# tudelft-iv/CCVPE

Measured on AMD Instinct MI355X. Metric: image-pairs/sec, higher is better.
Workload: dtype f32

## Files before the change

### ccvpe_amd/csrc/tail512.hip

```cpp
#include "conv_common.h"

namespace ccvpe {

struct TailParams {
  const void* x;
  const void* w;
  const float* shift9;
  const float* w2;
  const float* b2;
  float* out;
  float* smx;
  int H1, W1, c0, ld0, Kpad, normalize;
  int tiles_x, tiles_y, tiles_total, tiles_per_wg;
};

template <typename T, int COUT, int NCH, int TY, int TX, int WPP, bool SPLIT = false, bool PERSIST = false>
struct TailGeom {
  static constexpr int NW = 4 * WPP;
  static constexpr int NTHR = 64 * NW;
  static constexpr int PW = TX + 1;
  static constexpr int P = (TY + 1) * PW;
  static constexpr int NTILE = (P + 15) / 16;
  static constexpr int TPW = (NTILE + WPP - 1) / WPP;
  static constexpr int HR = TY + 2, HC = TX + 2, HPX = HR * HC;
  static constexpr bool WIDE_SLOT = TY == 8 && TX == 16 && (SPLIT || sizeof(T) == 2);
  static constexpr int LD = WIDE_SLOT ? 24 : 20;
  static constexpr int HCP = WIDE_SLOT ? 25 : HC;
  static constexpr int XBUF = HR * HCP * LD;
  static constexpr int NXB = NCH > 1 ? 2 : 1;
  static constexpr int SH = 2 * TY + 2, SW = 2 * TX + 2, SPL = SH * SW;
  static constexpr int NPL = 10;
  static constexpr int MAIN = (NXB * XBUF > NPL * SPL) ? NXB * XBUF : NPL * SPL;
  static constexpr int LDS_BYTES = (MAIN + 9 * 16) * 4;
  static constexpr int NOUT = (4 * TY * TX) / NTHR;
};

__device__ __forceinline__ void split4(f32x4 v, bf16x4& hi, bf16x4& lo) {
#pragma unroll
  for (int i = 0; i < 4; ++i) {
    hi[i] = (bf16_t)v[i];
    lo[i] = (bf16_t)(v[i] - (float)hi[i]);
  }
}

template <typename T, int COUT, int NCH, int TY, int TX, int WPP, bool SPLIT, bool PERSIST>
__global__ __launch_bounds__(256 * WPP, 2) void tail512_kernel(const TailParams p) {
  static_assert(!SPLIT || sizeof(T) == 4, "SPLIT reads fp32 operands");
  using G = TailGeom<T, COUT, NCH, TY, TX, WPP, SPLIT, PERSIST>;
  constexpr int E = ElemTraits<T>::E;
  constexpr int SK = 4 * E;
  constexpr int NTHR = G::NTHR, PW = G::PW, P = G::P, TPW = G::TPW;
  constexpr int HC = G::HC, HCP = G::HCP, HPX = G::HPX, LD = G::LD, XBUF = G::XBUF;
  constexpr int SW = G::SW, SPL = G::SPL;
  constexpr int H_IT = (HPX * 4 + NTHR - 1) / NTHR;
  static_assert((4 * TY * TX) % NTHR == 0, "stage 3 hands every thread the same number of outputs");

  extern __shared__ __attribute__((aligned(16))) float t5_sm[];
  float* Xs = t5_sm;
  float* Sp = t5_sm;
  float* Sh9 = t5_sm + G::MAIN;

  const int tid = threadIdx.x;
  const int lane = tid & 63;
  const int wave = sgpr(tid >> 6);
  const int par = wave & 3, wsub = wave >> 2;
  const int py = par >> 1, px = par & 1;
  const int pix = lane & 15, q = lane >> 4;

  const int wg = xcd_tile(blockIdx.x, gridDim.x);
  const int t_begin = wg * p.tiles_per_wg;
  const int t_end = min(t_begin + p.tiles_per_wg, p.tiles_total);
  const int tiles_xy = p.tiles_x * p.tiles_y;
  int b, y0, x0;
  auto tile_coords = [&](int t, int& tb, int& ty0, int& tx0) {
    tb = t / tiles_xy;
    const int r = t - tb * tiles_xy;
    const int ty = r / p.tiles_x;
    ty0 = ty * TY;
    tx0 = (r - ty * p.tiles_x) * TX;
  };
  const int H2 = 2 * p.H1, W2 = 2 * p.W1;
  const T* xg = reinterpret_cast<const T*>(p.x);

  for (int i = tid; i < 9 * 16; i += NTHR) Sh9[i] = p.shift9[i];

  constexpr int NWR = SPLIT ? 2 : 1;
  f32x4 wr[4][NCH][NWR];
  if constexpr (!SPLIT) {
    const T* wp = reinterpret_cast<const T*>(p.w) + ((size_t)par * 16 + pix) * p.Kpad;
#pragma unroll
    for (int tap = 0; tap < 4; ++tap)
#pragma unroll
      for (int c = 0; c < NCH; ++c) {
        const int ch = c * SK + q * E;
        wr[tap][c][0] = *reinterpret_cast<const f32x4*>(wp + (ch < p.c0 ? tap * p.c0 + ch : 0));
      }
#pragma unroll
    for (int tap = 0; tap < 4; ++tap)
#pragma unroll
      for (int c = 0; c < NCH; ++c) wr[tap][c][0] = keep_if(wr[tap][c][0], c * SK + q * E < p.c0);
  } else {
    const float* wp = reinterpret_cast<const float*>(p.w) + ((size_t)par * 16 + pix) * p.Kpad;
#pragma unroll
    for (int tap = 0; tap < 4; ++tap)
#pragma unroll
      for (int c = 0; c < NCH; ++c) {
        const int ch = c * 16 + (q & 1) * 8;
        const bool ok = ch < p.c0;
        const f32x4 v0 = keep_if(*reinterpret_cast<const f32x4*>(wp + (ok ? tap * p.c0 + ch : 0)), ok);
        const f32x4 v1 = keep_if(*reinterpret_cast<const f32x4*>(wp + (ok ? tap * p.c0 + ch + 4 : 0)), ok);
        bf16x4 h0, l0, h1, l1;
        split4(v0, h0, l0);
        split4(v1, h1, l1);
        bf16x8 hi, lo;
#pragma unroll
        for (int i = 0; i < 4; ++i) { hi[i] = h0[i]; hi[i + 4] = h1[i]; lo[i] = l0[i]; lo[i + 4] = l1[i]; }
        wr[tap][c][0] = __builtin_bit_cast(f32x4, hi);
        wr[tap][c][1] = keep_if(__builtin_bit_cast(f32x4, lo), q < 2);
      }
  }
  f32x4 w2f[COUT];
#pragma unroll
  for (int o = 0; o < COUT; ++o) {
    w2f[o] = keep_if(*reinterpret_cast<const f32x4*>(p.w2 + (o * 9 + min(pix, 8)) * 16 + q * 4), pix < 9);
  }

  const int hsub = tid & 3;
  int tidv = tid;
  f32x4 h_reg[H_IT];
  unsigned h_keep = 0;
  const int ld0s = sgpr(p.ld0);
  auto load_halo = [&](int c, int hb, int hy0, int hx0) {
    const int ch = c * SK + hsub * E;
    h_keep = 0;
#pragma unroll
    for (int it = 0; it < H_IT; ++it) {
      const int pxl = (tidv + NTHR * it) >> 2;
      const int hy = pxl / HC, hx = pxl - hy * HC;
      const int iy = hy0 - 1 + hy, ix = hx0 - 1 + hx;
      const bool ok = pxl < HPX && (unsigned)iy < (unsigned)p.H1 && (unsigned)ix < (unsigned)p.W1 && ch < p.c0;
      h_reg[it] = *reinterpret_cast<const f32x4*>(xg + (ok ? (size_t)((hb * p.H1 + iy) * p.W1 + ix) * ld0s + ch : 0));
      h_keep |= ok ? (1u << it) : 0u;
    }
  };
  auto store_halo = [&](int buf) {
#pragma unroll
    for (int it = 0; it < H_IT; ++it) {
      const int pxl = (tidv + NTHR * it) >> 2;
      const int slot = HCP == HC ? pxl : (pxl / HC) * HCP + (pxl % HC);
      const f32x4 v = keep_if(h_reg[it], (h_keep >> it) & 1u);
      if constexpr (!SPLIT) {
        if (pxl < HPX) *reinterpret_cast<f32x4*>(Xs + buf * XBUF + slot * LD + hsub * 4) = v;
      } else {
        bf16x4 hi, lo;
        split4(v, hi, lo);
        if (pxl < HPX) {
          float* row = Xs + buf * XBUF + slot * LD;
          *reinterpret_cast<bf16x4*>(reinterpret_cast<bf16_t*>(row) + hsub * 4) = hi;
          *reinterpret_cast<bf16x4*>(reinterpret_cast<bf16_t*>(row) + 16 + hsub * 4) = lo;
        }
      }
    }
  };

  if (t_begin >= t_end) return;
  tile_coords(t_begin, b, y0, x0);
  load_halo(0, b, y0, x0);
  for (int t = t_begin; t < t_end; ++t) {
  asm volatile("v_mov_b32 %0, %0" : "+v"(tidv));
  const int pixv = tidv & 15, qv = (tidv >> 4) & 3;
  int fbase[TPW];
#pragma unroll
  for (int i = 0; i < TPW; ++i) {
    const int pc = min((wsub * TPW + i) * 16 + pixv, P - 1);
    const int iy = pc / PW, ix = pc - iy * PW;
    fbase[i] = (iy * HCP + ix) * LD + qv * 4;
  }
  f32x4 acc[TPW];
#pragma unroll
  for (int i = 0; i < TPW; ++i) acc[i] = (f32x4){0.f, 0.f, 0.f, 0.f};

  store_halo(0);
  __syncthreads();
  constexpr int NPAIR = (TPW + 1) / 2, NS = NPAIR * 4;
#pragma unroll
  for (int c = 0; c < NCH; ++c) {
    if (c + 1 < NCH) load_halo(c + 1, b, y0, x0);
    __builtin_amdgcn_sched_barrier(0);
    const float* xb = Xs + (c & 1) * XBUF;
    f32x4 fr[2][2];
    auto read_step = [&](int s, f32x4* dst) {
      const int g = s >> 2, tap = s & 3;
      const int toff = ((tap >> 1) * HCP + (tap & 1)) * LD;
      dst[0] = *reinterpret_cast<const f32x4*>(xb + fbase[2 * g] + toff);
      if (2 * g + 1 < TPW) dst[1] = *reinterpret_cast<const f32x4*>(xb + fbase[2 * g + 1] + toff);
    };
    read_step(0, fr[0]);
#pragma unroll
    for (int s = 0; s < NS; ++s) {
      const int g = s >> 2, tap = s & 3;
      if (s + 1 < NS) read_step(s + 1, fr[(s + 1) & 1]);
      __builtin_amdgcn_sched_barrier(0);
      const f32x4 wv = wr[tap][c][0];
      const f32x4 f0 = fr[s & 1][0], f1 = fr[s & 1][1];
      if constexpr (SPLIT) {
#pragma unroll
        for (int h = 0; h < 2; ++h) {
          acc[2 * g] = mfma_stage<bf16_t>(wr[tap][c][h], f0, acc[2 * g]);
          if (2 * g + 1 < TPW) acc[2 * g + 1] = mfma_stage<bf16_t>(wr[tap][c][h], f1, acc[2 * g + 1]);
        }
      } else if constexpr (sizeof(T) == 4) {
#pragma unroll
        for (int kk = 0; kk < 4; ++kk) {
          acc[2 * g] = __builtin_amdgcn_mfma_f32_16x16x4f32(wv[kk], f0[kk], acc[2 * g], 0, 0, 0);
          if (2 * g + 1 < TPW) acc[2 * g + 1] = __builtin_amdgcn_mfma_f32_16x16x4f32(wv[kk], f1[kk], acc[2 * g + 1], 0, 0, 0);
        }
      } else {
        acc[2 * g] = mfma_stage<T>(wv, f0, acc[2 * g]);
        if (2 * g + 1 < TPW) acc[2 * g + 1] = mfma_stage<T>(wv, f1, acc[2 * g + 1]);
      }
      __builtin_amdgcn_sched_barrier(0);
    }
    if (c + 1 < NCH) {
      store_halo((c + 1) & 1);
      __syncthreads();
    }
  }
  if constexpr (PERSIST) {
    int nb, ny0, nx0;
    tile_coords(min(t + 1, t_end - 1), nb, ny0, nx0);
    load_halo(0, nb, ny0, nx0);
  }
  __syncthreads();
  __builtin_amdgcn_sched_barrier(0);

#pragma unroll
  for (int i = 0; i < TPW; ++i) {
    const int pc = min((wsub * TPW + i) * 16 + pixv, P - 1);
    const int iy = pc / PW, ix = pc - iy * PW;
    const int Y = 2 * (y0 + iy) - py, X = 2 * (x0 + ix) - px;
    const bool inside = (unsigned)Y < (unsigned)H2 && (unsigned)X < (unsigned)W2;
    const int rc = Y <= 0 ? 0 : (Y >= H2 - 1 ? 2 : 1);
    const int cc = X <= 0 ? 0 : (X >= W2 - 1 ? 2 : 1);
    const f32x4 sh = *reinterpret_cast<const f32x4*>(Sh9 + (rc * 3 + cc) * 16 + qv * 4);
#pragma unroll
    for (int r = 0; r < 4; ++r) acc[i][r] = inside ? fmaxf(acc[i][r] + sh[r], 0.f) : 0.f;
  }
  float res[COUT][G::NOUT];
#pragma unroll
  for (int o = 0; o < COUT; ++o) {
#pragma unroll
    for (int i = 0; i < TPW; ++i) {
      f32x4 s = {0.f, 0.f, 0.f, 0.f};
#pragma unroll
      for (int r = 0; r < 4; ++r) s = __builtin_amdgcn_mfma_f32_16x16x4f32(w2f[o][r], acc[i][r], s, 0, 0, 0);
      const int pt = (wsub * TPW + i) * 16 + pixv;
      const int iy = pt / PW, ix = pt - iy * PW;
      float* dst = Sp + (2 * iy + 1 - py) * SW + (2 * ix + 1 - px);
      if (pt < P) {
#pragma unroll
        for (int r = 0; r < 4; ++r) dst[min(4 * qv + r, 9) * SPL] = s[r];
      }
    }
    __syncthreads();
#pragma unroll
    for (int k = 0; k < G::NOUT; ++k) {
      const int e = tidv + NTHR * k;
      const int Yo = e / (2 * TX), Xo = e - Yo * (2 * TX);
      float v = p.b2[o];
#pragma unroll
      for (int t = 0; t < 9; ++t) v += Sp[t * SPL + (Yo + t / 3) * SW + Xo + t % 3];
      res[o][k] = v;
    }
    if (o + 1 < COUT) __syncthreads();
  }
#pragma unroll
  for (int k = 0; k < G::NOUT; ++k) {
    const int e = tidv + NTHR * k;
    const int Yo = e / (2 * TX), Xo = e - Yo * (2 * TX);
    if (COUT == 2 && p.normalize) {
      const float n = fmaxf(sqrtf(res[0][k] * res[0][k] + res[COUT - 1][k] * res[COUT - 1][k]), 1e-12f);
      res[0][k] /= n;
      res[COUT - 1][k] /= n;
    }
#pragma unroll
    for (int o = 0; o < COUT; ++o)
      p.out[((size_t)(b * COUT + o) * H2 + 2 * y0 + Yo) * W2 + 2 * x0 + Xo] = res[o][k];
  }
  if (COUT == 1 && p.smx) {
    float m = res[0][0];
#pragma unroll
    for (int k = 1; k < G::NOUT; ++k) m = fmaxf(m, res[0][k]);
    m = wave_max(m);
    float e = 0.f;
#pragma unroll
    for (int k = 0; k < G::NOUT; ++k) e += expf(res[0][k] - m);
    e = wave_sum(e);
    if (lane == 0) {
      float* dst = p.smx + ((size_t)t * G::NW + wave) * 2;
      dst[0] = m;
      dst[1] = e;
    }
  }
  if constexpr (!PERSIST) break;
  tile_coords(min(t + 1, t_end - 1), b, y0, x0);
  __syncthreads();
  }
}

template <typename T, int COUT, int NCH, int TY, int TX, int WPP, bool SPLIT = false, bool PERSIST = false>
static int launch_tail(const TailParams& p0, int batch, hipStream_t stream) {
  using G = TailGeom<T, COUT, NCH, TY, TX, WPP, SPLIT, PERSIST>;
  TailParams p = p0;
  if (p.W1 % TX || p.H1 % TY) return fail(CCVPE_EINVAL, "tail512: %d x %d is not a multiple of the %d x %d tile", p.H1, p.W1, TY, TX);
  p.tiles_x = p.W1 / TX;
  p.tiles_y = p.H1 / TY;
  const long total = (long)p.tiles_x * p.tiles_y * batch;
  if (total <= 0 || total > 0x7fffffffL) return fail(CCVPE_EINVAL, "tail512: bad grid");
  p.tiles_total = (int)total;
  const int max_wgs = 256 * 2 * 8;
  p.tiles_per_wg = PERSIST ? (int)((total + max_wgs - 1) / max_wgs) : 1;
  const int wgs = (int)((total + p.tiles_per_wg - 1) / p.tiles_per_wg);
  static bool attr_set = false;
  if (!attr_set) {
    hipError_t e = hipFuncSetAttribute((const void*)tail512_kernel<T, COUT, NCH, TY, TX, WPP, SPLIT, PERSIST>,
                                       hipFuncAttributeMaxDynamicSharedMemorySize, G::LDS_BYTES);
    if (e != hipSuccess) return fail(CCVPE_ELAUNCH, "tail512: set smem attr: %s", hipGetErrorString(e));
    attr_set = true;
  }
  hipLaunchKernelGGL((tail512_kernel<T, COUT, NCH, TY, TX, WPP, SPLIT, PERSIST>), dim3(wgs), dim3(G::NTHR), G::LDS_BYTES, stream, p);
  return check_launch("tail512_kernel");
}

template <typename T>
static int tail_any(const ccvpe_tail_desc* d, void* stream) {
  constexpr int E = ElemTraits<T>::E;
  constexpr int SK = 4 * E;
  if (!d) return fail(CCVPE_EINVAL, "tail512: null desc");
  if (d->c0 <= 0 || d->c0 % 8 || d->ld0 % E || d->ld0 < d->c0) return fail(CCVPE_EINVAL, "tail512: c0 %% 8, ld0 %% %d, ld0 >= c0 required", E);
  if (d->kpad < 4 * d->c0) return fail(CCVPE_EINVAL, "tail512: kpad %d < 4 * c0", d->kpad);
  if (d->cout != 1 && d->cout != 2) return fail(CCVPE_EINVAL, "tail512: cout must be 1 or 2");
  if (!d->x || !d->w || !d->shift9 || !d->w2 || !d->b2 || !d->out) return fail(CCVPE_EINVAL, "tail512: null pointer");
  if (!aligned16(d->x) || !aligned16(d->w) || !aligned16(d->w2) || !aligned16(d->shift9))
    return fail(CCVPE_EINVAL, "tail512: pointers must be 16-byte aligned");
  if (d->batch <= 0 || d->h1 <= 0 || d->w1 <= 0 || (long)d->batch * d->h1 * d->w1 > 0x1fffffffL) return fail(CCVPE_EINVAL, "tail512: bad shape");
  if (d->h1 % 16 || d->w1 % 16) return fail(CCVPE_EINVAL, "tail512: h1 and w1 must be multiples of 16 (got %d x %d)", d->h1, d->w1);
  TailParams p;
  p.x = d->x; p.w = d->w; p.shift9 = d->shift9; p.w2 = d->w2; p.b2 = d->b2; p.out = d->out;
  p.smx = d->cout == 1 ? d->softmax_partial : nullptr;
  p.H1 = d->h1; p.W1 = d->w1; p.c0 = d->c0; p.ld0 = d->ld0; p.Kpad = d->kpad; p.normalize = d->normalize;
  p.tiles_x = p.tiles_y = p.tiles_total = p.tiles_per_wg = 0;
  const int nch = (d->c0 + SK - 1) / SK;
  hipStream_t st = (hipStream_t)stream;
#define CCVPE_TAIL(COUT_, NCH_)                                                                                \
  if (d->cout == COUT_ && nch == NCH_) {                                                                       \
    if constexpr (sizeof(T) == 4) return launch_tail<T, COUT_, NCH_, 16, 16, 1, false, false>(p, d->batch, st); \
    else return launch_tail<T, COUT_, NCH_, 8, 16, 1, false, true>(p, d->batch, st);                           \
  }
  if constexpr (sizeof(T) == 4) {
    if (d->split) {
      if (d->cout == 1 && nch == 2) return launch_tail<T, 1, 2, 8, 16, 1, true, true>(p, d->batch, st);
      if (d->cout == 1 && nch == 3) return launch_tail<T, 1, 3, 8, 16, 1, true, true>(p, d->batch, st);
      return fail(CCVPE_EINVAL, "tail512: split mode is instantiated for cout 1, 17..48 channels");
    }
    CCVPE_TAIL(1, 2) CCVPE_TAIL(1, 3) CCVPE_TAIL(2, 2)
  } else {
    if (d->split) return fail(CCVPE_EINVAL, "tail512: split mode takes fp32 operands");
    CCVPE_TAIL(1, 1) CCVPE_TAIL(1, 2) CCVPE_TAIL(2, 1)
  }
#undef CCVPE_TAIL
  return fail(CCVPE_EINVAL, "tail512: (cout %d, c0 %d) not instantiated (fp32: cout 1 with c0 <= 48, cout 2 with c0 <= 32; bf16: cout 1 "
                            "with c0 <= 64, cout 2 with c0 <= 32)", d->cout, d->c0);
}

template <typename T>
static int tail_partials(const ccvpe_tail_desc* d) {
  if (!d || d->h1 <= 0 || d->w1 <= 0) return fail(CCVPE_EINVAL, "tail512_partials: bad desc");
  const bool small = sizeof(T) == 2 || d->split;
  const int ty = small ? 8 : 16;
  if (d->h1 % ty || d->w1 % 16) return fail(CCVPE_EINVAL, "tail512_partials: shape not tiled");
  return (d->h1 / ty) * (d->w1 / 16) * 4;
}

}

using namespace ccvpe;

extern "C" int ccvpe_tail512_partials(const ccvpe_tail_desc* desc, int is_bf16) {
  return is_bf16 ? tail_partials<bf16_t>(desc) : tail_partials<float>(desc);
}
extern "C" int ccvpe_tail512_f32(const ccvpe_tail_desc* desc, void* stream) { return tail_any<float>(desc, stream); }
extern "C" int ccvpe_tail512_bf16(const ccvpe_tail_desc* desc, void* stream) { return tail_any<bf16_t>(desc, stream); }
```

### ccvpe_amd/models.py

```python
import torch
import torch.nn as nn

from . import ops
from .synth import B0_BLOCKS, MODEL_SPECS, state_dict_spec

BN_EPS = 1e-3
SKIP_BLOCKS = (15, 10, 4, 2, 0)
MATCH_STRIDES = {"vigor": (64, 32, 16, 8, 4, 2),
                 "kitti": (128, 64, 32, 16, 8, 8),
                 "oxford": (64, 32, 16, 8, 4, 2)}


def window_offset(kind, channels, length):
    return int(channels / 2 - length / 2) if kind == "oxford" else 0


def _round_up(v, m):
    return (v + m - 1) // m * m


class _Holder(nn.Module):

    def forward(self, *a, **k):
        raise RuntimeError("parameter holder is not callable; use the owning CVM_* module")
# ... 59 lines not shown
def _pack_encoder(sd, p, dtype=torch.float32, fold_bn=True):
    fold = _fold_bn if fold_bn else (lambda _sd, _p: (None, None))
    e = _Obj()
    e.stem_w = sd[p + "._conv_stem.weight"].permute(2, 3, 1, 0).contiguous()
    e.stem_scale, e.stem_shift = fold(sd, p + "._bn0")
    e.blocks = []
    for i, (k, s, ex, cin, cout) in enumerate(B0_BLOCKS):
        b = _Obj()
        bp = "%s._blocks.%d" % (p, i)
        b.k, b.s, b.expand, b.cin, b.cout, b.mid = k, s, ex != 1, cin, cout, cin * ex
        if b.expand:
            b.w_exp = _pack_conv(sd[bp + "._expand_conv.weight"], dtype)
            b.s0, b.b0 = fold(sd, bp + "._bn0")
        b.w_dw = sd[bp + "._depthwise_conv.weight"].reshape(b.mid, k, k).permute(1, 2, 0).contiguous()
        b.s1, b.b1 = fold(sd, bp + "._bn1")
        b.se_w1 = sd[bp + "._se_reduce.weight"].reshape(-1, b.mid).contiguous()
        b.se_b1 = sd[bp + "._se_reduce.bias"].contiguous()
        b.se_w2 = sd[bp + "._se_expand.weight"].reshape(b.mid, -1).t().contiguous()
        b.se_b2 = sd[bp + "._se_expand.bias"].contiguous()
        b.w_proj = _pack_conv(sd[bp + "._project_conv.weight"], dtype)
        b.s2, b.b2 = fold(sd, bp + "._bn2")
        b.skip = (s == 1 and cin == cout)
        e.blocks.append(b)
    e.w_head = _pack_conv(sd[p + "._conv_head.weight"], dtype)
    e.head_scale, e.head_shift = fold(sd, p + "._bn1")
    return e


def _pack_deconv(w, bias, col_map, ldo, dtype=torch.float32):
    cin, cout = w.shape[0], w.shape[1]
    wg = w.permute(2, 3, 1, 0).reshape(4 * cout, cin)
    out = w.new_zeros((4 * cout, ldo))
    for d0, s0, n in col_map:
        out[:, d0:d0 + n] = wg[:, s0:s0 + n]
    return _pad2(out, dtype), bias.repeat(4).contiguous()


_UP_S = {0: {0: ((0, 1),), 1: ((1, 0), (2, 1))}, 1: {0: ((0, 0), (1, 1)), 1: ((2, 0),)}}
_UP_R = {0: (1, 2), 1: (0, 1, 2), 2: (0, 1)}
_OVERLAP_ENV = __import__("os").environ.get("CCVPE_OVERLAP_DECODERS", "auto")


OVERLAP_DECODERS_MAX_BATCH = 128


def _overlap_decoders(precision, batch=1):
    return _OVERLAP_ENV == "1" or (_OVERLAP_ENV == "auto" and precision == "bf16" and batch <= OVERLAP_DECODERS_MAX_BATCH)
FOLD_LEVELS = tuple(int(c) for c in __import__("os").environ.get("CCVPE_FOLD_LEVELS", "012345"))
FOLD_MIN_PIXELS = int(__import__("os").environ.get("CCVPE_FOLD_MIN_PIXELS", "2048"))
FUSE_TAIL = __import__("os").environ.get("CCVPE_FUSE_TAIL", "1") != "0"
SPLIT_TAIL = __import__("os").environ.get("CCVPE_SPLIT_TAIL", "1") != "0"
WINO = __import__("os").environ.get("CCVPE_WINO", "1") != "0"
SPLIT3 = __import__("os").environ.get("CCVPE_SPLIT3", "1") != "0"
SPLIT3_MIN_OK = 2
PACK_GRAPH = __import__("os").environ.get("CCVPE_PACK_GRAPH", "1") != "0"
PACK_GATHER = __import__("os").environ.get("CCVPE_PACK_GATHER", "1") != "0"
FUSE_MATCH = __import__("os").environ.get("CCVPE_FUSE_MATCH", "1") != "0"
FUSE_STEM = __import__("os").environ.get("CCVPE_FUSE_STEM", "1") != "0"
EVAL_TWO_STREAMS = __import__("os").environ.get("CCVPE_EVAL_TWO_STREAMS", "1") != "0"


def _pack_upconv(wd, bd, col_map, cp, w3, b3, dtype=torch.float32):
    cd, co = wd.shape[1], w3.shape[0]
    c1 = w3.shape[1] - cd
    wd_my = wd.new_zeros((cp, cd, 2, 2), dtype=torch.float64)
    for d0, s0, n in col_map:
        wd_my[d0:d0 + n] = wd[s0:s0 + n].double()
    w3d = w3[:, :cd].double()
    k = 4 * cp + 9 * c1
    kmult = 16 if dtype == torch.float32 else 32
    out = wd.new_zeros((4, _round_up(co, 16), _round_up(k, kmult)), dtype=torch.float64)
    for py in range(2):
        for px in range(2):
            par = py * 2 + px
            for du in range(2):
                for dv in range(2):
                    weff = wd.new_zeros((co, cp), dtype=torch.float64)
                    for ky, a in _UP_S[py][du]:
                        for kx, b in _UP_S[px][dv]:
                            weff += w3d[:, :, ky, kx] @ wd_my[:, :, a, b].t()
                    tap = du * 2 + dv
                    out[par, :co, tap * cp:(tap + 1) * cp] = weff
            if c1:
                out[par, :co, 4 * cp:k] = w3[:, cd:].double().permute(0, 2, 3, 1).reshape(co, 9 * c1)
    shift9 = wd.new_zeros((9, co), dtype=torch.float64)
    for rc in range(3):
        for cc in range(3):
            v = b3.double().clone()
            for ky in _UP_R[rc]:
                for kx in _UP_R[cc]:
                    v += w3d[:, :, ky, kx] @ bd.double()
            shift9[rc * 3 + cc] = v
    return out.to(dtype).contiguous(), shift9.float().contiguous()


def _split3_bf16(v):
    hi = v.to(torch.bfloat16)
    r = v - hi.float()
    mid = r.to(torch.bfloat16)
    lo = (r - mid.float()).to(torch.bfloat16)
    return hi, mid, lo


def _pack_upconv_s3(fw, cp, c1, dtype=torch.float32):
    if dtype != torch.float32 or fw is None or fw.dtype != torch.float32 or c1 <= 0:
        return None
    npad = fw.shape[1]
    nb0, nb1 = (cp + 15) // 16, (c1 + 15) // 16
    a = fw.new_zeros((4, npad, 4, nb0 * 16))
    a[..., :cp] = fw[:, :, :4 * cp].reshape(4, npad, 4, cp)
    a = a.reshape(4, npad, 4, nb0, 16).permute(0, 3, 2, 1, 4).reshape(4, 4 * nb0, npad, 16)
    s = fw.new_zeros((4, npad, 9, nb1 * 16))
# ... 258 lines not shown
            if gp is not None and gp[0] == where:
                self._pack_cache = gp[1].run()
            else:
                plan = repack.build(sd, pack)
                if plan is None:
                    self._pack_plan, self._pack_plan_failed = None, True
                    return self._packed()
                self._pack_plan = (where, plan)
                self._pack_cache = plan.pk
        elif self.training and PACK_GRAPH:
            where = (self.precision, self.fp32_tail_levels) + tuple(
                t.data_ptr() for t in list(self.parameters()) + list(self.buffers()))
            g = getattr(self, "_pack_graph", None)
            if g is not None and g[0] == where:
                g[1].replay()
                self._pack_cache = g[2]
            elif getattr(self, "_pack_where", None) == where and not getattr(self, "_pack_graph_failed", False):
                try:
                    graph = torch.cuda.CUDAGraph()
                    with torch.cuda.graph(graph, capture_error_mode="thread_local"):
                        pk = pack()
                    graph.replay()
                    self._pack_graph = (where, graph, pk)
                    self._pack_cache = pk
                except Exception:
                    self._pack_graph, self._pack_graph_failed = None, True
                    self._pack_cache = pack()
            else:
                self._pack_graph = None
                self._pack_where = where
                self._pack_cache = pack()
        else:
            self._pack_cache = pack()
        self._pack_key = key
        return self._pack_cache

    def _side_stream(self, which=1):
        dev = next(self.parameters()).device
        streams = self.__dict__.setdefault("_side_streams", {})
        st = streams.get(which)
        if st is None or st.device != dev:
            st = torch.cuda.Stream(device=dev)
            streams[which] = st
        return st

    def _ori_decoder(self, pk, cat6, sfeats, batch):
        xo = cat6
        normalize = not getattr(self, "ori_raw_output", False)
        for j in range(6):
            ov = pk.ori[j]
            hw = xo.shape[1]
            skip = sfeats[SKIP_BLOCKS[j]] if j < 5 else None
            if j == 5 and FUSE_TAIL and j in FOLD_LEVELS and ops.tail512_ok(hw, hw, ov.n_a):
                return ops.tail512(xo, ov.k, ov.fw, ov.fshift, ov.w_b, ov.b_b, 2, normalize, batch=batch, h1=hw, w1=hw)
            if j in FOLD_LEVELS and batch * hw * hw >= FOLD_MIN_PIXELS:
                y = _upconv_a(ov, xo, ov.k, batch, hw, skip)
            else:
                up = ops.conv_igemm(xo, ov.k, ov.up_w, ov.up_n, batch=batch, in_h=hw, in_w=hw,
                                    shift=ov.up_b, out_mode=ops.OUT_DECONV2X, algo_k=ov.k_algo)
                y = _double_conv(ov, up, skip, batch, 2 * hw)
            if j < 5:
                xo = _conv_b(ov, y, batch, 2 * hw)
            else:
                return ops.head_conv3x3(y, ov.w_b, ov.b_b, 2, normalize)

    def _loc_shifts(self):
        n_rot = MODEL_SPECS[self.kind]["n_rot"]
        if self.ori_noise is None:
            return list(range(n_rot))
        k = int(self.ori_noise / 18)
        return list(range(-k, k + 1))

    drop_connect_rate = 0.2
    BN_MOMENTUM = 0.01

    def forward(self, grd, sat, drop_masks=None):
        if self.training and self.precision != "fp32":
            raise NotImplementedError("ccvpe_amd: train mode is fp32 only")
        if not (grd.is_cuda and sat.is_cuda):
            raise RuntimeError("ccvpe_amd runs on the MI355X only: inputs must be device tensors")
        if self.training:
            from . import train
            if torch.is_grad_enabled() and any(p.requires_grad for p in self.parameters()):
                outs = train.apply(self, grd, sat, drop_masks)
            else:
                with torch.no_grad():
                    outs, _ = train.forward_train(self, grd, sat, drop_masks, rec=False)
            outs = list(outs)
            if self.ori_noise is not None:
                outs[3] = outs[3][:, len(self._loc_shifts()):]
            return tuple(outs)
        main = torch.cuda.current_stream()
        return self._forward_eval(grd, sat, main, self._side_stream() if EVAL_TWO_STREAMS else main)

    def _forward_eval(self, grd, sat, main, side):
        spec = MODEL_SPECS[self.kind]
        n_rot = spec["n_rot"]
        strides = MATCH_STRIDES[self.kind]
        circular = bool(self.circular_padding) and self.kind == "vigor"
        with torch.no_grad():
            pk = self._packed()
            grd = grd.contiguous().float()
            sat = sat.contiguous().float()
            batch = grd.shape[0]

            side.wait_stream(main)
            with torch.cuda.stream(side):
# ... 6 lines not shown
                                    shift=pk.gd_bias, ldd=_round_up(pk.gd_n, 4), out_f32=True)
                gdesc = ops.ground_descriptor(y1, pk.gd_wh, pk.gd_bh, spec["cd"])
            svol, sfeats = _run_encoder(pk.sat, sat, False, True, pk.dtype)
            main.wait_stream(side)
            gdesc.record_stream(main)
            sdesc = ops.conv_igemm(svol, 1280, pk.sd_w, pk.sd_n, batch=batch, in_h=svol.shape[1],
                                   in_w=svol.shape[2], kh=2, kw=2, stride=2, shift=pk.sd_bias)

            overlap = _overlap_decoders(self.precision, batch)
            loc_shifts = self._loc_shifts()
            fused = None
            scores_out = []
            smx = None
            x = sdesc
            cat6 = None
            goff = 0
            sfeats_loc = sfeats
            for j in range(6):
                lv = pk.loc[j]
                if j == pk.f32_from:
                    x = ops.cast_f32(x)
                    sfeats_loc = dict((SKIP_BLOCKS[q], ops.cast_f32(sfeats[SKIP_BLOCKS[q]])) for q in range(j, 5))
                hw = x.shape[1]
                cd = spec["cd"][j]
                L = gw * cd
                g = gdesc[:, goff:goff + L]
                goff += L
                if j == 0:
                    if self.ori_noise is None:
                        shifts, n_max = list(range(n_rot)), n_rot
                    else:
                        shifts, n_max = loc_shifts + list(range(n_rot)), len(loc_shifts)
                    n_tail = n_rot
                else:
                    shifts, n_max, n_tail = loc_shifts, len(loc_shifts), 0
                if fused is not None:
                    sc, cat = fused
                    fused = None
                else:
                    sc, cat = ops.match_level(x, g, L, shifts, n_max, n_tail, strides[j], lv.ldo, channels=lv.c,
                                              window_offset=window_offset(self.kind, lv.c, L))
                if j == 0:
                    cat6 = cat
                    scores_out.append(sc if self.ori_noise is None else sc[:, n_max:])
                    if overlap:
                        side.wait_stream(main)
                        with torch.cuda.stream(side):
                            x_ori = self._ori_decoder(pk, cat6, sfeats, batch)
                else:
                    scores_out.append(sc)
                skip = sfeats_loc[SKIP_BLOCKS[j]] if j < 5 else None
                if j == 5 and FUSE_TAIL and j in FOLD_LEVELS and ops.tail512_ok(hw, hw, lv.n_a):
                    logits_map, smx = ops.tail512(cat, lv.ldo, lv.fw, lv.fshift, lv.w_b, lv.b_b, 1, False, batch=batch, h1=hw, w1=hw,
                                                  split=(self.precision == "bf16" and cat.dtype == torch.float32 and SPLIT_TAIL),
                                                  want_softmax=True)
                    break
                if j in FOLD_LEVELS and batch * hw * hw >= FOLD_MIN_PIXELS:
                    y = _upconv_a(lv, cat, lv.ldo, batch, hw, skip)
                else:
                    up = ops.conv_igemm(cat, lv.ldo, lv.up_w, lv.up_n, batch=batch, in_h=hw, in_w=hw,
                                        shift=lv.up_b, out_mode=ops.OUT_DECONV2X, algo_k=lv.c + 1)
                    y = _double_conv(lv, up, skip, batch, 2 * hw)
                if j < 5:
                    to_f32 = j + 1 == pk.f32_from and y.dtype != torch.float32
                    nxt = pk.loc[j + 1]
                    L_n = gw * spec["cd"][j + 1]
                    if (FUSE_MATCH and len(loc_shifts) == 1 and
                            ops.conv3x3_match1(y, lv.n_a, lv.w_b, lv.n_b, None, L_n, loc_shifts[0], strides[j + 1], nxt.ldo, batch=batch,
                                               in_h=2 * hw, in_w=2 * hw, bias=lv.b_b, out_f32=to_f32, query_only=True)):
                        fused = ops.conv3x3_match1(y, lv.n_a, lv.w_b, lv.n_b, gdesc[:, goff:goff + L_n], L_n, loc_shifts[0],
                                                   strides[j + 1], nxt.ldo, batch=batch, in_h=2 * hw, in_w=2 * hw, bias=lv.b_b,
                                                   window_offset=window_offset(self.kind, nxt.c, L_n), out_f32=to_f32)
                        x = fused[1]
                    else:
                        x = _conv_b(lv, y, batch, 2 * hw, out_f32=to_f32)
                else:
                    logits_map = ops.head_conv3x3(y, lv.w_b, lv.b_b, 1, False)
            logits = logits_map.reshape(batch, -1)
            if smx is not None:
                heatmap = ops.softmax_apply(logits, smx).reshape(logits_map.shape)
            else:
                heatmap = ops.softmax_rows(logits).reshape(logits_map.shape)

            if overlap:
                main.wait_stream(side)
                x_ori.record_stream(main)
            else:
                x_ori = self._ori_decoder(pk, cat6, sfeats, batch)
        return (logits, heatmap, x_ori) + tuple(scores_out)


class CVM_VIGOR(_CVMBase):
    kind = "vigor"

    def __init__(self, device, circular_padding, efficientnet_weights=None):
        super().__init__(device, circular_padding, None, efficientnet_weights)


class CVM_VIGOR_ori_prior(_CVMBase):
    kind = "vigor"

    def __init__(self, device, ori_noise, circular_padding=True, efficientnet_weights=None):
        super().__init__(device, circular_padding, ori_noise, efficientnet_weights)


class CVM_OxfordRobotCar(_CVMBase):
    kind = "oxford"
# ... 11 lines not shown
```

### ccvpe_amd/ops.py

```python
import ctypes

import torch

from . import _lib
from ._lib import ConvDesc, check

ACT_NONE, ACT_RELU, ACT_SWISH, ACT_RELU_MASK = 0, 1, 2, 3
SPLIT_K_CALLS = 0
SPLIT_K = __import__("os").environ.get("CCVPE_SPLIT_K", "1") == "1"
OUT_NHWC, OUT_DECONV2X = 0, 1

_recorder = None


def set_recorder(rec):
    global _recorder
    _recorder = rec


class LaunchRecorder(object):

    def __init__(self):
        self.items = []

# ... 286 lines not shown
    ld0 = ld0 if ld0 is not None else src0.shape[-1]
    ld1 = ld1 if ld1 is not None else (src1.shape[-1] if src1 is not None else 0)
    d = _s3_desc(src0, c0, w3_packed, None, n, batch, h1, w1, src1, c1, ACT_NONE, None, ldd if ldd is not None else n, ld0, ld1)
    return int(_lib.load().ccvpe_upconv3x3_s3_form_ok(ctypes.byref(d), form))


def upconv3x3_s3(src0, c0, w3_packed, shift9, n, *, batch, h1, w1, src1=None, c1=0, act=ACT_NONE, dst=None, ldd=None, ld0=None,
                 ld1=None, form=None):
    lib = _lib.load()
    for t, nm in ((src0, "src0"), (src1, "src1"), (shift9, "shift9"), (dst, "dst")):
        _chk(t, nm)
    _chk(w3_packed, "w", torch.bfloat16)
    ld0 = ld0 if ld0 is not None else src0.shape[-1]
    ld1 = ld1 if ld1 is not None else (src1.shape[-1] if src1 is not None else 0)
    if dst is None:
        ldd = ldd if ldd is not None else n
        dst = _empty((batch, 2 * h1, 2 * w1, ldd), device=src0.device)
    elif ldd is None:
        ldd = dst.shape[-1]
    d = _s3_desc(src0, c0, w3_packed, shift9, n, batch, h1, w1, src1, c1, act, dst, ldd, ld0, ld1)
    rec = _recorder
    ev0 = rec.begin() if rec is not None else None
    if form is None:
        check(lib.ccvpe_upconv3x3_s3_f32(ctypes.byref(d), _stream()), "ccvpe_upconv3x3_s3_f32")
    else:
        check(lib.ccvpe_upconv3x3_s3_form_f32(ctypes.byref(d), form, _stream()), "ccvpe_upconv3x3_s3_form_f32")
    if rec is not None:
        m = batch * h1 * w1 * 4
        k_eff = 4 * c0 + 9 * c1
        flops = 2.0 * m * n * k_eff
        nbytes = 4.0 * (batch * h1 * w1 * c0 + m * c1 + m * n + 4 * n * k_eff)
        tile = igemm_tile(n).split("<")[1]
        name = "upconv_s3_kernel<%s%s" % (tile[:-1], ",pair>" if (h1 == 8 and w1 == 8) else ">")
        if lib.ccvpe_upconv3x3_s3_form_ok(ctypes.byref(d), form or 0) == 2:
            name = "upconv_s3q_kernel<2,%d>" % ((n + 15) // 16)
        rec.end(name, "up3x3 M%d N%d Keff%d" % (m, n, k_eff), flops, nbytes, ev0)
    return dst


def tail512(x, c0, w_packed, shift9, w2, b2, cout, normalize, *, batch, h1, w1, split=False, want_softmax=False):
    lib = _lib.load()
    dt = _act_dtype(x)
    _chk(x, "x", dt)
    _chk(w_packed, "w", dt)
    for t, nm in ((shift9, "shift9"), (w2, "w2"), (b2, "b2")):
        _chk(t, nm)
    if tuple(w2.shape) != (cout, 3, 3, 16) or tuple(shift9.shape) != (9, 16) or w_packed.shape[0] != 4 or w_packed.shape[1] != 16:
        raise ValueError("tail512: w [4,16,kpad], shift9 [9,16], w2 [cout,3,3,16] expected")
    out = _empty((batch, cout, 2 * h1, 2 * w1), device=x.device, dtype=torch.float32)
    d = _lib.TailDesc()
    d.x, d.w, d.shift9, d.w2, d.b2, d.out = _ptr(x), _ptr(w_packed), _ptr(shift9), _ptr(w2), _ptr(b2), _ptr(out)
    d.batch, d.h1, d.w1 = batch, h1, w1
    d.c0, d.ld0, d.kpad = c0, x.shape[-1], w_packed.shape[-1]
    d.cout, d.normalize, d.split = cout, int(bool(normalize)), int(bool(split))
    smx = None
    if want_softmax:
        npart = lib.ccvpe_tail512_partials(ctypes.byref(d), int(dt != torch.float32))
        if npart <= 0:
            check(int(npart) if npart < 0 else -1, "ccvpe_tail512_partials")
        smx = _empty((batch, npart, 2), device=x.device, dtype=torch.float32)
        d.softmax_partial = _ptr(smx)
    rec = _recorder
    ev0 = rec.begin() if rec is not None else None
    fn = lib.ccvpe_tail512_f32 if dt == torch.float32 else lib.ccvpe_tail512_bf16
    check(fn(ctypes.byref(d), _stream()), "ccvpe_tail512")
    if rec is not None:
        m = batch * h1 * w1 * 4
        esz = 4.0 if dt == torch.float32 else 2.0
        rec.end("tail512_kernel<%s,%d>" % (("f32" if not split else "f32 as bf16 hi+lo") if dt == torch.float32 else "bf16", cout), "tail M%d Keff%d" % (m, 4 * c0),
                2.0 * m * 16 * (4 * c0 + 9 * cout), esz * batch * h1 * w1 * c0 + 4.0 * m * cout, ev0)
    return (out, smx) if want_softmax else out


def softmax_apply(logits, partials):
    lib = _lib.load()
    _chk(logits, "logits")
    _chk(partials, "partials")
    rows, n = logits.shape
    out = _empty(logits.shape, device=logits.device, dtype=logits.dtype)
    check(lib.ccvpe_softmax_apply_f32(_ptr(logits), _ptr(partials), partials.shape[1], _ptr(out), rows, n, _stream()),
          "ccvpe_softmax_apply_f32")
    return out


def tail512_ok(h1, w1, n_a):
    return n_a == 16 and h1 % 16 == 0 and w1 % 16 == 0


def stem_conv(x_nchw, w, scale, shift, circular, out_dtype=torch.float32):
    lib = _lib.load()
    for t, nm in ((x_nchw, "x"), (w, "w"), (scale, "scale"), (shift, "shift")):
        _chk(t, nm)
    b, c, h, wd = x_nchw.shape
    if c != 3:
        raise ValueError("stem expects 3 input channels")
    ho, wo = (h + 1 - 3) // 2 + 1, (wd + 1 - 3) // 2 + 1
    y = _empty((b, ho, wo, 32), device=x_nchw.device, dtype=out_dtype)
    fn = lib.ccvpe_stem_conv_f32 if out_dtype == torch.float32 else lib.ccvpe_stem_conv_bf16
    check(fn(_ptr(x_nchw), _ptr(w), _ptr(scale), _ptr(shift), _ptr(y), b, h, wd, int(bool(circular)), _stream()),
          "ccvpe_stem_conv")
    return y


def stem_dw_supported(in_h, in_w, circular):
    return _lib.load().ccvpe_stem_dw_nblk(in_h, in_w, int(bool(circular)))


def stem_dw(x_nchw, w, s0, b0, w_dw, s1, b1, circular, out_dtype=torch.float32):
    lib = _lib.load()
    for t, nm in ((x_nchw, "x"), (w, "w"), (s0, "s0"), (b0, "b0"), (w_dw, "w_dw"), (s1, "s1"), (b1, "b1")):
        _chk(t, nm)
    b, c, h, wd = x_nchw.shape
    if c != 3 or w_dw.numel() != 9 * 32:
        raise ValueError("stem_dw expects 3 input channels and a 3x3x32 depthwise weight")
    nblk = stem_dw_supported(h, wd, circular)
    if nblk <= 0:
        raise _lib.CcvpeError("stem_dw: unsupported shape %s" % (tuple(x_nchw.shape),))
    ho, wo = (h + 1 - 3) // 2 + 1, (wd + 1 - 3) // 2 + 1
    y = _empty((b, ho, wo, 32), device=x_nchw.device, dtype=out_dtype)
    part = _empty((b, nblk, 32), device=x_nchw.device, dtype=torch.float32)
    rec = _recorder
    ev0 = rec.begin() if rec is not None else None
# ... 299 lines not shown
```

Before: 2686.

## Add three-plane bf16 split mode to fused fp32 tail512 kernel

Adds a SPLIT=3 variant of the tail kernel that splits fp32 activations and weights into hi/mid/lo bf16 planes and runs bf16 MFMAs instead of fp32 MFMAs. The aim is fp32-level accuracy at bf16 matrix-core throughput. It is enabled by default for fp32-precision models in both the orientation and localization tail calls. To save registers, w2 weights are staged through LDS instead of held per thread. The costs are extra MFMA passes, extra conversion work and more LDS.

```diff
diff --git a/ccvpe_amd/csrc/tail512.hip b/ccvpe_amd/csrc/tail512.hip
--- a/ccvpe_amd/csrc/tail512.hip
+++ b/ccvpe_amd/csrc/tail512.hip
@@ -14,7 +14,7 @@
   int tiles_x, tiles_y, tiles_total, tiles_per_wg;
 };
 
-template <typename T, int COUT, int NCH, int TY, int TX, int WPP, bool SPLIT = false, bool PERSIST = false>
+template <typename T, int COUT, int NCH, int TY, int TX, int WPP, int SPLIT = 0, bool PERSIST = false>
 struct TailGeom {
   static constexpr int NW = 4 * WPP;
   static constexpr int NTHR = 64 * NW;
@@ -23,7 +23,8 @@
   static constexpr int NTILE = (P + 15) / 16;
   static constexpr int TPW = (NTILE + WPP - 1) / WPP;
   static constexpr int HR = TY + 2, HC = TX + 2, HPX = HR * HC;
-  static constexpr bool WIDE_SLOT = TY == 8 && TX == 16 && (SPLIT || sizeof(T) == 2);
+  static constexpr bool WIDE_SLOT = TY == 8 && TX == 16 && (SPLIT != 0 || sizeof(T) == 2);
+  static_assert(SPLIT != 3 || WIDE_SLOT, "three planes need the 96-byte slot");
   static constexpr int LD = WIDE_SLOT ? 24 : 20;
   static constexpr int HCP = WIDE_SLOT ? 25 : HC;
   static constexpr int XBUF = HR * HCP * LD;
@@ -31,7 +32,8 @@
   static constexpr int SH = 2 * TY + 2, SW = 2 * TX + 2, SPL = SH * SW;
   static constexpr int NPL = 10;
   static constexpr int MAIN = (NXB * XBUF > NPL * SPL) ? NXB * XBUF : NPL * SPL;
-  static constexpr int LDS_BYTES = (MAIN + 9 * 16) * 4;
+  static constexpr int W2S = SPLIT == 3 ? COUT * 9 * 16 : 0;
+  static constexpr int LDS_BYTES = (MAIN + 9 * 16 + W2S) * 4;
   static constexpr int NOUT = (4 * TY * TX) / NTHR;
 };
 
@@ -43,8 +45,19 @@
   }
 }
 
-template <typename T, int COUT, int NCH, int TY, int TX, int WPP, bool SPLIT, bool PERSIST>
+__device__ __forceinline__ void split4x3(f32x4 v, bf16x4& hi, bf16x4& mid, bf16x4& lo) {
+#pragma unroll
+  for (int i = 0; i < 4; ++i) {
+    hi[i] = (bf16_t)v[i];
+    const float r = v[i] - (float)hi[i];
+    mid[i] = (bf16_t)r;
+    lo[i] = (bf16_t)(r - (float)mid[i]);
+  }
+}
+
+template <typename T, int COUT, int NCH, int TY, int TX, int WPP, int SPLIT, bool PERSIST>
 __global__ __launch_bounds__(256 * WPP, 2) void tail512_kernel(const TailParams p) {
+  static_assert(SPLIT == 0 || SPLIT == 2 || SPLIT == 3, "SPLIT is a plane count");
   static_assert(!SPLIT || sizeof(T) == 4, "SPLIT reads fp32 operands");
   using G = TailGeom<T, COUT, NCH, TY, TX, WPP, SPLIT, PERSIST>;
   constexpr int E = ElemTraits<T>::E;
@@ -83,6 +96,9 @@
   const T* xg = reinterpret_cast<const T*>(p.x);
 
   for (int i = tid; i < 9 * 16; i += NTHR) Sh9[i] = p.shift9[i];
+  [[maybe_unused]] float* W2s = Sh9 + 9 * 16;
+  if constexpr (SPLIT == 3)
+    for (int i = tid; i < G::W2S; i += NTHR) W2s[i] = p.w2[i];
 
   constexpr int NWR = SPLIT ? 2 : 1;
   f32x4 wr[4][NCH][NWR];
@@ -109,6 +125,21 @@
         const bool ok = ch < p.c0;
         const f32x4 v0 = keep_if(*reinterpret_cast<const f32x4*>(wp + (ok ? tap * p.c0 + ch : 0)), ok);
         const f32x4 v1 = keep_if(*reinterpret_cast<const f32x4*>(wp + (ok ? tap * p.c0 + ch + 4 : 0)), ok);
+        if constexpr (SPLIT == 3) {
+          bf16x4 h0, m0, l0, h1, m1, l1;
+          split4x3(v0, h0, m0, l0);
+          split4x3(v1, h1, m1, l1);
+          bf16x8 f0, f1;
+#pragma unroll
+          for (int i = 0; i < 4; ++i) {
+            f0[i] = q < 2 ? h0[i] : m0[i];
+            f0[i + 4] = q < 2 ? h1[i] : m1[i];
+            f1[i] = q < 2 ? h0[i] : l0[i];
+            f1[i + 4] = q < 2 ? h1[i] : l1[i];
+          }
+          wr[tap][c][0] = __builtin_bit_cast(f32x4, f0);
+          wr[tap][c][1] = __builtin_bit_cast(f32x4, f1);
+        } else {
         bf16x4 h0, l0, h1, l1;
         split4(v0, h0, l0);
         split4(v1, h1, l1);
@@ -117,12 +148,15 @@
         for (int i = 0; i < 4; ++i) { hi[i] = h0[i]; hi[i + 4] = h1[i]; lo[i] = l0[i]; lo[i + 4] = l1[i]; }
         wr[tap][c][0] = __builtin_bit_cast(f32x4, hi);
         wr[tap][c][1] = keep_if(__builtin_bit_cast(f32x4, lo), q < 2);
+        }
       }
   }
   f32x4 w2f[COUT];
-#pragma unroll
-  for (int o = 0; o < COUT; ++o) {
-    w2f[o] = keep_if(*reinterpret_cast<const f32x4*>(p.w2 + (o * 9 + min(pix, 8)) * 16 + q * 4), pix < 9);
+  if constexpr (SPLIT != 3) {
+#pragma unroll
+    for (int o = 0; o < COUT; ++o) {
+      w2f[o] = keep_if(*reinterpret_cast<const f32x4*>(p.w2 + (o * 9 + min(pix, 8)) * 16 + q * 4), pix < 9);
+    }
   }
 
   const int hsub = tid & 3;
@@ -151,6 +185,15 @@
       const f32x4 v = keep_if(h_reg[it], (h_keep >> it) & 1u);
       if constexpr (!SPLIT) {
         if (pxl < HPX) *reinterpret_cast<f32x4*>(Xs + buf * XBUF + slot * LD + hsub * 4) = v;
+      } else if constexpr (SPLIT == 3) {
+        bf16x4 hi, mid, lo;
+        split4x3(v, hi, mid, lo);
+        if (pxl < HPX) {
+          bf16_t* row = reinterpret_cast<bf16_t*>(Xs + buf * XBUF + slot * LD);
+          *reinterpret_cast<bf16x4*>(row + hsub * 4) = hi;
+          *reinterpret_cast<bf16x4*>(row + 16 + hsub * 4) = mid;
+          *reinterpret_cast<bf16x4*>(row + 32 + hsub * 4) = lo;
+        }
       } else {
         bf16x4 hi, lo;
         split4(v, hi, lo);
@@ -174,8 +217,9 @@
   for (int i = 0; i < TPW; ++i) {
     const int pc = min((wsub * TPW + i) * 16 + pixv, P - 1);
     const int iy = pc / PW, ix = pc - iy * PW;
-    fbase[i] = (iy * HCP + ix) * LD + qv * 4;
-  }
+    fbase[i] = (iy * HCP + ix) * LD + (SPLIT == 3 ? qv & 1 : qv) * 4;
+  }
+  [[maybe_unused]] const int f3off = qv < 2 ? 16 : 0;
   f32x4 acc[TPW];
 #pragma unroll
   for (int i = 0; i < TPW; ++i) acc[i] = (f32x4){0.f, 0.f, 0.f, 0.f};
@@ -195,6 +239,28 @@
       dst[0] = *reinterpret_cast<const f32x4*>(xb + fbase[2 * g] + toff);
       if (2 * g + 1 < TPW) dst[1] = *reinterpret_cast<const f32x4*>(xb + fbase[2 * g + 1] + toff);
     };
+    if constexpr (SPLIT == 3) {
+      constexpr int NU = NS * 3;
+      f32x4 fb[3][2];
+      auto read_sub = [&](int u, f32x4* dst) {
+        const int g = u / 12, tap = (u / 3) & 3, h = u % 3;
+        const int toff = ((tap >> 1) * HCP + (tap & 1)) * LD + (h == 1 ? 8 : 0);
+        const int lane_off = h == 2 ? f3off : 0;
+        dst[0] = *reinterpret_cast<const f32x4*>(xb + fbase[2 * g] + lane_off + toff);
+        if (2 * g + 1 < TPW) dst[1] = *reinterpret_cast<const f32x4*>(xb + fbase[2 * g + 1] + lane_off + toff);
+      };
+      read_sub(0, fb[0]);
+      read_sub(1, fb[1]);
+#pragma unroll
+      for (int u = 0; u < NU; ++u) {
+        const int g = u / 12, tap = (u / 3) & 3, h = u % 3;
+        if (u + 2 < NU) read_sub(u + 2, fb[(u + 2) % 3]);
+        __builtin_amdgcn_sched_barrier(0);
+        acc[2 * g] = mfma_stage<bf16_t>(wr[tap][c][h >> 1], fb[u % 3][0], acc[2 * g]);
+        if (2 * g + 1 < TPW) acc[2 * g + 1] = mfma_stage<bf16_t>(wr[tap][c][h >> 1], fb[u % 3][1], acc[2 * g + 1]);
+        __builtin_amdgcn_sched_barrier(0);
+      }
+    } else {
     read_step(0, fr[0]);
 #pragma unroll
     for (int s = 0; s < NS; ++s) {
@@ -203,7 +269,7 @@
       __builtin_amdgcn_sched_barrier(0);
       const f32x4 wv = wr[tap][c][0];
       const f32x4 f0 = fr[s & 1][0], f1 = fr[s & 1][1];
-      if constexpr (SPLIT) {
+      if constexpr (SPLIT == 2) {
 #pragma unroll
         for (int h = 0; h < 2; ++h) {
           acc[2 * g] = mfma_stage<bf16_t>(wr[tap][c][h], f0, acc[2 * g]);
@@ -220,6 +286,7 @@
         if (2 * g + 1 < TPW) acc[2 * g + 1] = mfma_stage<T>(wv, f1, acc[2 * g + 1]);
       }
       __builtin_amdgcn_sched_barrier(0);
+    }
     }
     if (c + 1 < NCH) {
       store_halo((c + 1) & 1);
@@ -247,6 +314,11 @@
     for (int r = 0; r < 4; ++r) acc[i][r] = inside ? fmaxf(acc[i][r] + sh[r], 0.f) : 0.f;
   }
   float res[COUT][G::NOUT];
+  if constexpr (SPLIT == 3) {
+#pragma unroll
+    for (int o = 0; o < COUT; ++o)
+      w2f[o] = keep_if(*reinterpret_cast<const f32x4*>(W2s + (o * 9 + min(pixv, 8)) * 16 + qv * 4), pixv < 9);
+  }
 #pragma unroll
   for (int o = 0; o < COUT; ++o) {
 #pragma unroll
@@ -308,7 +380,7 @@
   }
 }
 
-template <typename T, int COUT, int NCH, int TY, int TX, int WPP, bool SPLIT = false, bool PERSIST = false>
+template <typename T, int COUT, int NCH, int TY, int TX, int WPP, int SPLIT = 0, bool PERSIST = false>
 static int launch_tail(const TailParams& p0, int batch, hipStream_t stream) {
   using G = TailGeom<T, COUT, NCH, TY, TX, WPP, SPLIT, PERSIST>;
   TailParams p = p0;
@@ -354,15 +426,22 @@
   hipStream_t st = (hipStream_t)stream;
 #define CCVPE_TAIL(COUT_, NCH_)                                                                                \
   if (d->cout == COUT_ && nch == NCH_) {                                                                       \
-    if constexpr (sizeof(T) == 4) return launch_tail<T, COUT_, NCH_, 16, 16, 1, false, false>(p, d->batch, st); \
-    else return launch_tail<T, COUT_, NCH_, 8, 16, 1, false, true>(p, d->batch, st);                           \
+    if constexpr (sizeof(T) == 4) return launch_tail<T, COUT_, NCH_, 16, 16, 1, 0, false>(p, d->batch, st); \
+    else return launch_tail<T, COUT_, NCH_, 8, 16, 1, 0, true>(p, d->batch, st);                           \
   }
   if constexpr (sizeof(T) == 4) {
-    if (d->split) {
-      if (d->cout == 1 && nch == 2) return launch_tail<T, 1, 2, 8, 16, 1, true, true>(p, d->batch, st);
-      if (d->cout == 1 && nch == 3) return launch_tail<T, 1, 3, 8, 16, 1, true, true>(p, d->batch, st);
-      return fail(CCVPE_EINVAL, "tail512: split mode is instantiated for cout 1, 17..48 channels");
-    }
+    if (d->split == 1) {
+      if (d->cout == 1 && nch == 2) return launch_tail<T, 1, 2, 8, 16, 1, 2, true>(p, d->batch, st);
+      if (d->cout == 1 && nch == 3) return launch_tail<T, 1, 3, 8, 16, 1, 2, true>(p, d->batch, st);
+      return fail(CCVPE_EINVAL, "tail512: split mode 1 is instantiated for cout 1, 17..48 channels");
+    }
+    if (d->split == 2) {
+      if (d->cout == 1 && nch == 2) return launch_tail<T, 1, 2, 8, 16, 1, 3, true>(p, d->batch, st);
+      if (d->cout == 1 && nch == 3) return launch_tail<T, 1, 3, 8, 16, 1, 3, true>(p, d->batch, st);
+      if (d->cout == 2 && nch == 2) return launch_tail<T, 2, 2, 8, 16, 1, 3, true>(p, d->batch, st);
+      return fail(CCVPE_EINVAL, "tail512: split mode 2 is instantiated for cout 1 with 17..48 channels and cout 2 with 17..32");
+    }
+    if (d->split) return fail(CCVPE_EINVAL, "tail512: split must be 0, 1 or 2 (got %d)", d->split);
     CCVPE_TAIL(1, 2) CCVPE_TAIL(1, 3) CCVPE_TAIL(2, 2)
   } else {
     if (d->split) return fail(CCVPE_EINVAL, "tail512: split mode takes fp32 operands");
diff --git a/ccvpe_amd/models.py b/ccvpe_amd/models.py
--- a/ccvpe_amd/models.py
+++ b/ccvpe_amd/models.py
@@ -135,12 +135,21 @@
 SPLIT_TAIL = __import__("os").environ.get("CCVPE_SPLIT_TAIL", "1") != "0"
 WINO = __import__("os").environ.get("CCVPE_WINO", "1") != "0"
 SPLIT3 = __import__("os").environ.get("CCVPE_SPLIT3", "1") != "0"
+SPLIT3_TAIL = SPLIT3 and __import__("os").environ.get("CCVPE_SPLIT3_TAIL", "1") != "0"
 SPLIT3_MIN_OK = 2
 PACK_GRAPH = __import__("os").environ.get("CCVPE_PACK_GRAPH", "1") != "0"
 PACK_GATHER = __import__("os").environ.get("CCVPE_PACK_GATHER", "1") != "0"
 FUSE_MATCH = __import__("os").environ.get("CCVPE_FUSE_MATCH", "1") != "0"
 FUSE_STEM = __import__("os").environ.get("CCVPE_FUSE_STEM", "1") != "0"
 EVAL_TWO_STREAMS = __import__("os").environ.get("CCVPE_EVAL_TWO_STREAMS", "1") != "0"
+
+
+def _tail_split(precision, x, cout):
+    if x.dtype != torch.float32:
+        return 0
+    if precision == "bf16":
+        return 1 if SPLIT_TAIL and cout == 1 else 0
+    return 2 if SPLIT3 and SPLIT3_TAIL else 0
 
 
 def _pack_upconv(wd, bd, col_map, cp, w3, b3, dtype=torch.float32):
@@ -505,7 +514,8 @@
             hw = xo.shape[1]
             skip = sfeats[SKIP_BLOCKS[j]] if j < 5 else None
             if j == 5 and FUSE_TAIL and j in FOLD_LEVELS and ops.tail512_ok(hw, hw, ov.n_a):
-                return ops.tail512(xo, ov.k, ov.fw, ov.fshift, ov.w_b, ov.b_b, 2, normalize, batch=batch, h1=hw, w1=hw)
+                return ops.tail512(xo, ov.k, ov.fw, ov.fshift, ov.w_b, ov.b_b, 2, normalize, batch=batch, h1=hw, w1=hw,
+                                   split=_tail_split(self.precision, xo, 2))
             if j in FOLD_LEVELS and batch * hw * hw >= FOLD_MIN_PIXELS:
                 y = _upconv_a(ov, xo, ov.k, batch, hw, skip)
             else:
@@ -618,7 +628,7 @@
                 skip = sfeats_loc[SKIP_BLOCKS[j]] if j < 5 else None
                 if j == 5 and FUSE_TAIL and j in FOLD_LEVELS and ops.tail512_ok(hw, hw, lv.n_a):
                     logits_map, smx = ops.tail512(cat, lv.ldo, lv.fw, lv.fshift, lv.w_b, lv.b_b, 1, False, batch=batch, h1=hw, w1=hw,
-                                                  split=(self.precision == "bf16" and cat.dtype == torch.float32 and SPLIT_TAIL),
+                                                  split=_tail_split(self.precision, cat, 1),
                                                   want_softmax=True)
                     break
                 if j in FOLD_LEVELS and batch * hw * hw >= FOLD_MIN_PIXELS:
diff --git a/ccvpe_amd/ops.py b/ccvpe_amd/ops.py
--- a/ccvpe_amd/ops.py
+++ b/ccvpe_amd/ops.py
@@ -362,7 +362,8 @@
     d.x, d.w, d.shift9, d.w2, d.b2, d.out = _ptr(x), _ptr(w_packed), _ptr(shift9), _ptr(w2), _ptr(b2), _ptr(out)
     d.batch, d.h1, d.w1 = batch, h1, w1
     d.c0, d.ld0, d.kpad = c0, x.shape[-1], w_packed.shape[-1]
-    d.cout, d.normalize, d.split = cout, int(bool(normalize)), int(bool(split))
+    split = int(split)
+    d.cout, d.normalize, d.split = cout, int(bool(normalize)), split
     smx = None
     if want_softmax:
         npart = lib.ccvpe_tail512_partials(ctypes.byref(d), int(dt != torch.float32))
@@ -377,7 +378,7 @@
     if rec is not None:
         m = batch * h1 * w1 * 4
         esz = 4.0 if dt == torch.float32 else 2.0
-        rec.end("tail512_kernel<%s,%d>" % (("f32" if not split else "f32 as bf16 hi+lo") if dt == torch.float32 else "bf16", cout), "tail M%d Keff%d" % (m, 4 * c0),
+        rec.end("tail512_kernel<%s,%d>" % (("f32", "f32 as bf16 hi+lo", "f32 as bf16 hi+mid+lo")[split] if dt == torch.float32 else "bf16", cout), "tail M%d Keff%d" % (m, 4 * c0),
                 2.0 * m * 16 * (4 * c0 + 9 * cout), esz * batch * h1 * w1 * c0 + 4.0 * m * cout, ev0)
     return (out, smx) if want_softmax else out
 
```

Result: faster. 2747 (median of 6 runs) (+2.3%).
